# dmar-bonn/ipp-rl

Measured on AMD Instinct MI355X. Metric: env-steps/s (batched) on 50x50 grid, higher is better.
Workload: dtype f32

## Files before the change

ipp-rl_amd/csrc/k_prepare.h:

```cpp
#pragma once
#include "ipp_common.h"

#ifndef IPP_PREP_MINWAVES
#define IPP_PREP_MINWAVES 4
#endif

namespace ipp {

__device__ inline double area_weight(int src, int dst, int d, int s) {
    const double scale = (double)src / (double)dst;
    const double a = d * scale, b = a + scale;
    const double cell = fmin(scale, (double)src - a);
    int s1 = (int)ceil(a);
    const int s2 = min((int)floor(b), src - 1);
    s1 = min(s1, s2);
    double w = 0.0;
    if (s == s1 - 1 && s1 - a > 1e-3) w += (double)(float)((s1 - a) / cell);
    if (s >= s1 && s < s2) w += (double)(float)(1.0 / cell);
    if (s == s2 && b - s2 > 1e-3) w += (double)(float)(fmin(fmin(b - s2, 1.0), cell) / cell);
    return w;
}

template <int MC>
__host__ __device__ constexpr size_t prep_small_bytes() {
// ... 472 lines not shown
    int status = h.status;
    int fallback = 0;

    if (pd) {
        if (tid < m) {
            const int j = tid;
            for (int i = 0; i < m; ++i) Li[i * LD + j] = 0.0;
            Li[j * LD + j] = 1.0 / L[j * LD + j];
            for (int i = j - 1; i >= 0; --i) {
                double s = 0.0;
                for (int k = i + 1; k <= j; ++k) s += L[k * LD + i] * Li[k * LD + j];
                Li[i * LD + j] = -s / L[i * LD + i];
            }
        }
        prep_sync<WAVE>();
        if (tid < m) {
            double s = 0.0;
            for (int i = 0; i <= tid; ++i) s += Li[i * LD + tid] * vv[i];
            yy[tid] = s;
        }
    } else if (MODE == IPP_DENSE) {
        fallback = 1;
        status = IPP_STATUS_CHOL_FALLBACK;
        if (tid == 0) {
            for (int i = 0; i < m; ++i)
                for (int j = 0; j < m; ++j) { L[i * LD + j] = S[i * LD + j]; Li[i * LD + j] = (i == j) ? 1.0 : 0.0; }
            for (int c = 0; c < m; ++c) {
                int piv = c;
                double best = fabs(L[c * LD + c]);
                for (int i = c + 1; i < m; ++i)
                    if (fabs(L[i * LD + c]) > best) { best = fabs(L[i * LD + c]); piv = i; }
                if (piv != c)
                    for (int j = 0; j < m; ++j) {
                        double t = L[c * LD + j]; L[c * LD + j] = L[piv * LD + j]; L[piv * LD + j] = t;
                        t = Li[c * LD + j]; Li[c * LD + j] = Li[piv * LD + j]; Li[piv * LD + j] = t;
                    }
                const double inv = 1.0 / L[c * LD + c];
                for (int j = 0; j < m; ++j) { L[c * LD + j] *= inv; Li[c * LD + j] *= inv; }
                for (int i = 0; i < m; ++i)
                    if (i != c) {
                        const double fct = L[i * LD + c];
                        if (fct != 0.0)
                            for (int j = 0; j < m; ++j) { L[i * LD + j] -= fct * L[c * LD + j]; Li[i * LD + j] -= fct * Li[c * LD + j]; }
                    }
            }
        }
        prep_sync<WAVE>();
        if (tid < m) {
            double s = 0.0;
            for (int i = 0; i < m; ++i) s += Li[tid * LD + i] * vv[i];
            yy[tid] = s;
        }
    } else {
        status = IPP_STATUS_NOT_PD;
    }
    prep_sync<WAVE>();
    IPP_TICK(v, 5, tick);

    if (WAVE && threadIdx.x == 0) IPP_MARK(item, 7);
    const bool dead = (MODE == IPP_FACTOR) && !pd;
    for (int idx = tid; idx < MC * MC; idx += kPrepThreads) {
        const int i = idx / MC, j = idx - i * MC;
        const double val = (!dead && i < m && j < m) ? Li[i * LD + j] : 0.0;
        linv_f[idx] = (float)val;
        if (linv_f2) linv_f2[idx] = (float)val;
        dbg[MC * MC + idx] = val;
        dbg[idx] = (i < m && j < m) ? S[i * LD + j] : 0.0;
    }
    for (int i = tid; i < MC; i += kPrepThreads) {
        const double yval = (!dead && !cov_only && i < m) ? yy[i] : 0.0;
        y_f[i] = (float)yval;
        if (y_f2) y_f2[i] = (float)yval;
        dbg[2 * MC * MC + i] = (i < m) ? zz[i] : 0.0;
        dbg[2 * MC * MC + MC + i] = yval;
    }
    constexpr int QS = (MC + 3) & ~3;
    constexpr int QP = (QS <= 16) ? 16 : 32;
    if (MODE == IPP_FACTOR) {
        const int j = tid & (QP - 1);
        if (j < QS) {
            for (int k = tid / QP; k < r; k += kPrepThreads / QP) {
                double sacc = 0.0;
                const int SI = (si > 0) ? si : ht_ld, SK = (si > 0) ? sk : 1;
                if (!dead && j < m)
                    for (int i = 0; i <= j; ++i) sacc += (double)big[i * SI + k * SK] * Li[i * LD + j];
                q_out[k * QS + j] = (float)(-sacc);
            }
        }
    } else {
        const int j = tid & (QP - 1);
        if (j < QS) {
            for (int fi = tid / QP; fi < f; fi += kPrepThreads / QP) {
                const int ly = fi / h.w, lx = fi - ly * h.w;
                const int bi = (ly / h.rf) * h.nx + lx / h.rf;
                double sacc = 0.0;
                if (j < m) sacc = fallback ? ((bi == j) ? bwt[bi] : 0.0) : bwt[bi] * Li[bi * LD + j];
                q_out[fi * QS + j] = (float)sacc;
            }
        }
    }
    {
        const int qrows = (MODE == IPP_FACTOR) ? r : f;
        for (int idx = tid; idx < 8 * QS; idx += kPrepThreads) q_out[(size_t)qrows * QS + idx] = 0.f;
    }
    if (tid == 0) {
        ItemHdr ho = h;
        ho.status = status;
        ho.fallback = fallback;
        if (dead) { ho.commit = 0; ho.rows = 0; }
        v.hdr[item] = ho;
        *hs = ho;
        if (status_out) status_out[item] = status;
    }
    IPP_TICK(v, 6, tick);
    return hs;
}

template <int MC, int MODE, int NT>
__device__ __forceinline__ ItemHdr* prepare_item(const View& v, const int item, const int* __restrict__ env_ids,
                                                 const int* __restrict__ dst_ids, const double* __restrict__ action,
                                                 const double* __restrict__ prev_action,
                                                 const float* __restrict__ meas_noise, unsigned flags,
                                                 int* __restrict__ status_out, float* __restrict__ obs_out,
                                                 int* __restrict__ obs_m, int* __restrict__ obs_shape,
                                                 unsigned char* small, float* big, int si, int sk, float* q_out,
                                                 float* linv_f, float* linv_f2, float* y_f, float* y_f2, int* span_s) {
    return prepare_item_ex<MC, MODE, NT, false>(v, item, env_ids, dst_ids, action, prev_action, meas_noise, flags, status_out,
                                                obs_out, obs_m, obs_shape, small, big, si, sk, q_out, linv_f, linv_f2, y_f,
                                                y_f2, span_s, NoMidWork());
}

__device__ __forceinline__ void wave_lds_sync() {
    __builtin_amdgcn_fence(__ATOMIC_ACQ_REL, "workgroup");
    __builtin_amdgcn_wave_barrier();
}

template <int MC>
__device__ __forceinline__ int solve_wave(const View& v, const ItemHdr& h, const int item, unsigned flags,
                                          unsigned char* small, const float* ht, float* linv_f, float* y_f,
                                          int* __restrict__ status_out) {
    constexpr int LD = MC + 1;
    constexpr int QS = (MC + 3) & ~3;
    const PrepLds<MC> pl(small);
    double* S = pl.S; double* L = pl.L; double* Li = pl.Li; double* zz = pl.zz; double* vv = pl.vv; double* yy = pl.yy;
    const double* ktab = pl.ktab; const int* bfi = pl.bfi; const int* bcnt = pl.bcnt; const double* bwt = pl.bwt;
    const int lane = threadIdx.x & (kWave - 1);
    const int m = h.m, r = h.rank;
    const double R = (double)(h.rf * h.rf * h.rf) * h.nv_d;
    const bool cov_only = (flags & IPP_COV_ONLY) != 0;
    double* dbg = v.dbg + (size_t)item * (2 * MC * MC + 2 * MC);

    {
        constexpr int GL = 8;
        const int grp = lane / GL, sl = lane & (GL - 1), n_grp = kWave / GL;
        const int npairs = m * (m + 1) / 2;
        for (int p0 = 0; p0 < npairs; p0 += n_grp) {
            const int p = p0 + grp;
            const bool on = p < npairs;
            int i = 0, j = 0;
            if (on) {
                j = (int)((sqrtf(8.0f * p + 1.0f) - 1.0f) * 0.5f);
                while (j * (j + 1) / 2 > p) --j;
                while ((j + 1) * (j + 2) / 2 <= p) ++j;
                i = p - j * (j + 1) / 2;
            }
            double acc = 0.0;
            if (on) {
                const int ci = bcnt[i], cj = bcnt[j];
                const int sh = (cj == 4) ? 2 : (cj == 2 ? 1 : 0);
                const double wij = bwt[i] * bwt[j];
                for (int c = sl; c < ci * cj; c += GL) {
                    const int fa = bfi[4 * i + (c >> sh)], fb = bfi[4 * j + (c & (cj - 1))];
                    acc += wij * ktab[abs(bfi_y(fa) - bfi_y(fb)) * h.w + abs(bfi_x(fa) - bfi_x(fb))];
                }
                for (int k = sl; k < r; k += GL) acc -= (double)ht[k * QS + i] * (double)ht[k * QS + j];
            }
#pragma unroll
            for (int off = GL / 2; off > 0; off >>= 1) acc += __shfl_xor(acc, off, GL);
            if (on && sl == 0) {
                if (i == j) acc += R;
                S[i * LD + j] = acc;
                S[j * LD + i] = acc;
            }
        }
    }
    wave_lds_sync();

    bool pd = true;
    for (int c = 0; c < m; ++c) {
        double d = 0.0;
        if (lane == 0) {
            d = S[c * LD + c];
            for (int k = 0; k < c; ++k) d -= L[c * LD + k] * L[c * LD + k];
            L[c * LD + c] = sqrt(d);
        }
        d = __shfl(d, 0, kWave);
        if (!(d > 0.0)) { pd = false; break; }
        wave_lds_sync();
        if (lane > c && lane < m) {
            double sacc = S[lane * LD + c];
            for (int k = 0; k < c; ++k) sacc -= L[lane * LD + k] * L[c * LD + k];
            L[lane * LD + c] = sacc / L[c * LD + c];
        }
        wave_lds_sync();
    }
    int status = h.status;
    if (pd) {
        if (lane < m) {
            const int j = lane;
            for (int i = 0; i < m; ++i) Li[i * LD + j] = 0.0;
            Li[j * LD + j] = 1.0 / L[j * LD + j];
            for (int i = j - 1; i >= 0; --i) {
                double sacc = 0.0;
                for (int k = i + 1; k <= j; ++k) sacc += L[k * LD + i] * Li[k * LD + j];
                Li[i * LD + j] = -sacc / L[i * LD + i];
            }
        }
        wave_lds_sync();
        if (lane < m) {
            double sacc = 0.0;
            for (int i = 0; i <= lane; ++i) sacc += Li[i * LD + lane] * vv[i];
            yy[lane] = sacc;
        }
        wave_lds_sync();
    } else {
        status = IPP_STATUS_NOT_PD;
    }
    const bool dead = !pd;
    for (int idx = lane; idx < MC * MC; idx += kWave) {
        const int i = idx / MC, j = idx - i * MC;
        const double val = (!dead && i < m && j < m) ? Li[i * LD + j] : 0.0;
        linv_f[idx] = (float)val;
        dbg[MC * MC + idx] = val;
        dbg[idx] = (i < m && j < m) ? S[i * LD + j] : 0.0;
    }
    for (int i = lane; i < MC; i += kWave) {
        const double yval = (!dead && !cov_only && i < m) ? yy[i] : 0.0;
        y_f[i] = (float)yval;
        dbg[2 * MC * MC + i] = (i < m) ? zz[i] : 0.0;
        dbg[2 * MC * MC + MC + i] = yval;
    }
    if (lane == 0) {
        ItemHdr ho = h;
        ho.status = status;
        ho.fallback = 0;
        if (dead) { ho.commit = 0; ho.rows = 0; }
        v.hdr[item] = ho;
        if (status_out) status_out[item] = status;
    }
    return status;
}

template <int MC>
__device__ __forceinline__ void observe_wave(const View& v, const ItemHdr& h, unsigned flags, unsigned char* small, const ObsRegs o) {
    const PrepLds<MC> pl(small);
    double* L = pl.L; double* zz = pl.zz; double* vv = pl.vv; double* sub = pl.sub;
    const int lane = threadIdx.x & (kWave - 1);
    const int m = h.m, f = h.f;
    const bool cov_only = (flags & IPP_COV_ONLY) != 0;
    if (cov_only) {
        if (lane < MC) { zz[lane] = 0.0; vv[lane] = 0.0; }
        wave_lds_sync();
        return;
    }
    float gt_f = o.gt;
    asm volatile("" : "+v"(gt_f));
    if (lane < f) sub[lane] = (double)gt_f;
    double* wyt = L;
    double* wxt = L + 2 * MC;
    if (h.rf > 1) {
        const int ocols = (h.h + h.rf - 1) / h.rf, orows = (h.w + h.rf - 1) / h.rf;
        for (int idx = lane; idx < orows * h.h; idx += kWave) wyt[idx] = area_weight(h.h, orows, idx / h.h, idx % h.h);
        for (int idx = lane; idx < ocols * h.w; idx += kWave) wxt[idx] = area_weight(h.w, ocols, idx / h.w, idx % h.w);
    }
    wave_lds_sync();
    if (lane < m) {
        const Block myb = block_of(lane, h.nx, h.rf, h.w, h.h);
        double val;
        if (h.rf == 1) {
            val = sub[lane];
        } else {
            const int ocols = (h.h + h.rf - 1) / h.rf;
            const int orow = lane / ocols, ocol = lane - orow * ocols;
            val = 0.0;
            for (int sy = 0; sy < h.h; ++sy) {
                const double wy = wyt[orow * h.h + sy];
                if (wy == 0.0) continue;
                for (int sx = 0; sx < h.w; ++sx) {
                    const double wx = wxt[ocol * h.w + sx];
                    if (wx != 0.0) val += sub[sy * h.w + sx] * wx * wy;
                }
            }
        }
        float eps_f = o.eps;
        asm volatile("" : "+v"(eps_f));
        const double eps = (double)eps_f;
        if (flags & IPP_GIVEN_OBSERVATION)
            val = eps;
        else
            val = fmin(fmax(val + h.nv_d * eps, 0.0), 1.0);
        zz[lane] = val;
        double hx = 0.0;
        const int cnt_b = myb.count();
#pragma unroll
        for (int a = 0; a < 4; ++a)
            if (a < cnt_b) hx += myb.weight * (double)o.mean[a];
        vv[lane] = val - hx;
    } else if (lane < MC) {
        zz[lane] = 0.0;
        vv[lane] = 0.0;
    }
    wave_lds_sync();
}


template <int MC>
__device__ __forceinline__ int solve_wave_fast(const View& v, const ItemHdr& h, const int item, unsigned flags,
                                               unsigned char* small, const float* ht, int si, int sk, float* linv_f,
                                               float* y_f, float* __restrict__ q_out, int* __restrict__ status_out,
                                               int* obs_flag = nullptr, int r_ht = -1, const float* ht2 = nullptr, int r_ht2 = 0) {
    static_assert(MC == 9, "register layout written for MC = 9");
    constexpr int LD = MC + 1;
    constexpr int QS = (MC + 3) & ~3;
    const PrepLds<MC> pl(small);
    double* S = pl.S; double* zz = pl.zz; double* vv = pl.vv;
    const double* ktab = pl.ktab; const int* bfi = pl.bfi; const int* bcnt = pl.bcnt; const double* bwt = pl.bwt;
    const int lane = threadIdx.x & (kWave - 1);
    const int m = h.m, r = r_ht >= 0 ? r_ht : h.rank;
    const double R = (double)(h.rf * h.rf * h.rf) * h.nv_d;
    const bool cov_only = (flags & IPP_COV_ONLY) != 0;
    double* dbg = v.dbg + (size_t)item * (2 * MC * MC + 2 * MC);

    int pi = 0, pj = 0;
    {
        int j = (int)((sqrtf(8.0f * lane + 1.0f) - 1.0f) * 0.5f);
        while (j * (j + 1) / 2 > lane) --j;
        while ((j + 1) * (j + 2) / 2 <= lane) ++j;
        pj = j;
        pi = lane - j * (j + 1) / 2;
    }
    const bool pair_on = pj < m;
    double mine = 0.0;
    if (pair_on) {
        const int ci = bcnt[pi], cj = bcnt[pj];
        const int sh = (cj == 4) ? 2 : (cj == 2 ? 1 : 0);
        const double wij = bwt[pi] * bwt[pj];
        for (int c = 0; c < ci * cj; ++c) {
            const int fa = bfi[4 * pi + (c >> sh)], fb = bfi[4 * pj + (c & (cj - 1))];
            mine += wij * ktab[abs(bfi_y(fa) - bfi_y(fb)) * h.w + abs(bfi_x(fa) - bfi_x(fb))];
        }
        if (pi == pj) mine += R;
    }
    if (pair_on) {
        const float* hi = ht + pi * si;
        const float* hj = ht + pj * si;
        double a0 = 0.0, a1 = 0.0, a2 = 0.0, a3 = 0.0;
        auto groups = [&](const float* xi, const float* xj, int n) {
            int k = 0;
            for (; k + 8 <= n; k += 8) {
                float x[8], y[8];
#pragma unroll
                for (int u = 0; u < 8; ++u) { x[u] = xi[(k + u) * sk]; y[u] = xj[(k + u) * sk]; }
                a0 = fma((double)x[0], (double)y[0], a0); a1 = fma((double)x[1], (double)y[1], a1);
                a2 = fma((double)x[2], (double)y[2], a2); a3 = fma((double)x[3], (double)y[3], a3);
                a0 = fma((double)x[4], (double)y[4], a0); a1 = fma((double)x[5], (double)y[5], a1);
                a2 = fma((double)x[6], (double)y[6], a2); a3 = fma((double)x[7], (double)y[7], a3);
            }
            for (; k < n; ++k) a0 = fma((double)xi[k * sk], (double)xj[k * sk], a0);
        };
        groups(hi, hj, r);
        if (ht2) groups(ht2 + pi * si, ht2 + pj * si, r_ht2);
        mine -= (a0 + a1) + (a2 + a3);
    }
    if (pair_on) {
        S[pi * LD + pj] = mine;
        S[pj * LD + pi] = mine;
    }
    wave_lds_sync();

    double c[MC];
#pragma unroll
    for (int k = 0; k < MC; ++k) c[k] = (lane < m && k < m) ? S[min(lane, MC - 1) * LD + k] : ((k == lane) ? 1.0 : 0.0);
    const bool capture = v.dbg_capture == 1;
    if (capture && lane < MC) {
#pragma unroll
        for (int k = 0; k < MC; ++k) dbg[lane * MC + k] = (lane < m && k < m) ? c[k] : 0.0;
    }
    bool pd = true;
    double rd[MC];
#pragma unroll
    for (int j = 0; j < MC; ++j) {
        rd[j] = 1.0;
        if (j < m) {
            double t = c[j];
#pragma unroll
            for (int k = 0; k < j; ++k) t = fma(-c[k], bcast_lane(c[k], j), t);
            const double d = bcast_lane(t, j);
            if (!(d > 0.0)) pd = false;
            double y = __builtin_amdgcn_rsq(d);
#pragma unroll
            for (int it = 0; it < 2; ++it) {
                const double e = fma(-(d * y), y, 1.0);
                y = fma(0.5 * y, e, y);
            }
            rd[j] = y;
            c[j] = (lane == j) ? d * y : t * y;
        }
    }
    int status = h.status;
    double li[MC];
#pragma unroll
    for (int i = 0; i < MC; ++i) li[i] = 0.0;
    if (pd) {
#pragma unroll
        for (int i = MC - 1; i >= 0; --i) {
            if (i < m) {
                double sacc = 0.0;
#pragma unroll
                for (int k = i + 1; k < MC; ++k) {
                    if (k < m) {
                        const double cki = bcast_lane(c[i], k);
                        if (k <= lane) sacc = fma(cki, li[k], sacc);
                    }
                }
                li[i] = (lane == i) ? rd[i] : ((lane > i && lane < m) ? -sacc * rd[i] : 0.0);
            }
        }
    } else {
        status = IPP_STATUS_NOT_PD;
    }
    const bool dead = !pd;
    if (obs_flag) {
        while (__hip_atomic_load(obs_flag, __ATOMIC_ACQUIRE, __HIP_MEMORY_SCOPE_WORKGROUP) == 0) __builtin_amdgcn_s_sleep(2);
    }
    double yv = 0.0;
    if (pd && lane < m) {
#pragma unroll
        for (int i = 0; i < MC; ++i)
            if (i <= lane) yv = fma(li[i], vv[i], yv);
    }
    if (lane < MC) {
#pragma unroll
        for (int i = 0; i < MC; ++i) {
            const double val = (!dead && i < m && lane < m) ? li[i] : 0.0;
            linv_f[i * MC + lane] = (float)val;
            if (capture) dbg[MC * MC + i * MC + lane] = val;
        }
        const double yval = (!dead && !cov_only && lane < m) ? yv : 0.0;
        y_f[lane] = (float)yval;
        if (capture) {
            dbg[2 * MC * MC + lane] = (lane < m) ? zz[lane] : 0.0;
            dbg[2 * MC * MC + MC + lane] = yval;
        }
    }
    if (lane == 0) {
        ItemHdr ho = h;
        ho.status = status;
        ho.fallback = 0;
        if (dead) { ho.commit = 0; ho.rows = 0; }
        v.hdr[item] = ho;
        *pl.hs = ho;
        if (status_out) status_out[item] = status;
    }
    wave_lds_sync();
    if (q_out) {
        for (int k0 = 0; k0 < r; k0 += kWave) {
            const int k = k0 + lane;
            if (k < r) {
                float hv[MC], q[QS];
#pragma unroll
                for (int i = 0; i < MC; ++i) hv[i] = (i < m) ? ht[i * si + k * sk] : 0.f;
#pragma unroll
                for (int j = 0; j < QS; ++j) {
                    float acc = 0.f;
                    if (j < MC) {
#pragma unroll
                        for (int i = 0; i <= j; ++i) acc = fmaf(hv[i], linv_f[i * MC + j], acc);
                    }
                    q[j] = -acc;
                }
                float4* dst = reinterpret_cast<float4*>(q_out + (size_t)k * QS);
#pragma unroll
                for (int j4 = 0; j4 < QS / 4; ++j4) dst[j4] = make_float4(q[4 * j4], q[4 * j4 + 1], q[4 * j4 + 2], q[4 * j4 + 3]);
            }
        }
        for (int idx = lane; idx < 8 * QS; idx += kWave) q_out[(size_t)r * QS + idx] = 0.f;
    }
    return status;
}

template <int MC, int MODE>
__global__ __launch_bounds__(kPrepThreads, IPP_PREP_MINWAVES) void k_prepare(View v, const int* __restrict__ env_ids,
                                                          const int* __restrict__ dst_ids, int n_items,
                                                          const double* __restrict__ action,
                                                          const double* __restrict__ prev_action,
                                                          const float* __restrict__ meas_noise, unsigned flags,
                                                          int* __restrict__ status_out, float* __restrict__ obs_out,
                                                          int* __restrict__ obs_m, int* __restrict__ obs_shape) {
    extern __shared__ __attribute__((aligned(16))) unsigned char smem[];
    if ((int)blockIdx.x >= n_items) return;
    const int item = launch_item(v, blockIdx.x, n_items);
    constexpr int LQ = (MC * MC + MC + 3) & ~3;
    float* blk_out = v.q + (size_t)item * v.q_item;
    float* big = reinterpret_cast<float*>(smem + ((prep_small_bytes<MC>() + 15) & ~(size_t)15));
    if constexpr (MC == 9 && MODE == IPP_FACTOR) {
        if (!obs_out) {
            ItemHdr* hs = prepare_item_ex<MC, MODE, kPrepThreads, true>(v, item, env_ids, dst_ids, action, prev_action, meas_noise, flags,
                                                                        status_out, nullptr, nullptr, nullptr, smem, big, 0, 1, nullptr,
                                                                        v.linv + (size_t)item * MC * MC, blk_out, v.yv + (size_t)item * MC,
                                                                        blk_out + MC * MC, nullptr, NoMidWork());
            if (threadIdx.x >= kWave) return;
            const ItemHdr h = uniform_hdr(*hs);
            if (h.m == 0) return;
            const PrepLds<MC> pl(smem);
            float* Ls = reinterpret_cast<float*>(pl.L);
            float* ys = Ls + MC * MC;
            solve_wave_fast<MC>(v, h, item, flags, smem, big, (h.rank + 3) & ~3, 1, Ls, ys, blk_out + LQ, status_out);
            wave_lds_sync();
            const int lane = threadIdx.x;
            for (int i = lane; i < MC * MC; i += kWave) { const float x = Ls[i]; v.linv[(size_t)item * MC * MC + i] = x; blk_out[i] = x; }
            if (lane < MC) { const float x = ys[lane]; v.yv[(size_t)item * MC + lane] = x; blk_out[MC * MC + lane] = x; }
            return;
        }
    }
    prepare_item<MC, MODE, kPrepThreads>(v, item, env_ids, dst_ids, action, prev_action, meas_noise, flags, status_out,
                                         obs_out, obs_m, obs_shape, smem, big, 0, 1, blk_out + LQ,
                                         v.linv + (size_t)item * MC * MC, blk_out, v.yv + (size_t)item * MC,
                                         blk_out + MC * MC, nullptr);
}

}
```

ipp-rl_amd/csrc/k_step_patch.h:

```cpp
#pragma once
#include <algorithm>
#include <cstdlib>
#include <type_traits>
#include "ipp_common.h"
#include "k_gain.h"
#include "k_gain_factor.h"
#include "k_prepare.h"

namespace ipp {

constexpr int kPatchRec = 16;
constexpr int kPatchKP = 8;
constexpr int kPatchRowAux = 2;
constexpr int kPatchStoreAux = IPP_NT_STORES ? 2 : 0;
constexpr int kPatchMinW = 6;
constexpr int kPatchWavesDefault = 3;
constexpr int kPatchWavesPerCu = 4 * kPatchMinW;
constexpr int kPatchCtl = 32;
constexpr int kPatchMaxRank = 512;

struct PatchGeo {
    int pw, ph, pstride, plw, punits;
};
inline PatchGeo patch_geometry(int W, int H, int R) {
    PatchGeo g;
    g.pw = std::min((W + 1) & ~1, ((2 * R + 5 + 2) / 2) * 2);
    g.ph = std::min(H, 2 * R + 6);
    g.pstride = (g.pw * g.ph + 15) & ~15;
    g.plw = std::min(std::max(W, H), R + 7);
    g.punits = (g.ph * g.pw + 2 * kWave - 1) / (2 * kWave);
    return g;
}

struct PatchLds {
    float* rec; float* Ls; float* ys; float* lut; unsigned char* small; double* red; int* ctl; int* fb_yx; float* fb_w;
    unsigned short* ridx; double* unit_red;
    static constexpr int LQ = 96;
    __host__ __device__ static size_t small_bytes() { return (prep_small_bytes<9>() + 15) & ~(size_t)15; }
    __host__ __device__ static size_t bytes(int cap, int lut_floats, int waves, int units, int rank_cap) {
        size_t b = (size_t)cap * kPatchRec * 4 + LQ * 4 + (size_t)((lut_floats + 3) & ~3) * 4 + small_bytes();
        b += 4 * 8 + kPatchCtl * 4 + 2 * 4 * 9 * 4;
        b += (((size_t)waves * (rank_cap + kPatchKP) * 2) + 15) & ~(size_t)15;
        b += (size_t)units * 8;
        return (b + 15) & ~(size_t)15;
    }
    __device__ __forceinline__ PatchLds(unsigned char* base, int cap, int lut_floats, int waves, int units, int rank_cap) {
        rec = reinterpret_cast<float*>(base);
        Ls = rec + (size_t)cap * kPatchRec;
        ys = Ls + 81;
        lut = Ls + LQ;
        small = reinterpret_cast<unsigned char*>(lut + ((lut_floats + 3) & ~3));
        red = reinterpret_cast<double*>(small + small_bytes());
        ctl = reinterpret_cast<int*>(red + 4);
        fb_yx = ctl + kPatchCtl;
        fb_w = reinterpret_cast<float*>(fb_yx + 4 * 9);
        ridx = reinterpret_cast<unsigned short*>(fb_w + 4 * 9);
        unit_red = reinterpret_cast<double*>(ridx + ((((size_t)waves * (rank_cap + kPatchKP)) + 7) & ~(size_t)7));
    }
};

}
#include "k_patch_units.h"
namespace ipp {

struct StepIo {
    static constexpr bool kMean = true;
    typedef float rowv __attribute__((ext_vector_type(2)));
    __amdgpu_buffer_rsrc_t row_rs;
    float* mean_rw;
    float* diag_rw;
    bool cov_only;
    int m, row0_bytes, pstride_bytes;
    __device__ __forceinline__ rowv row_load(unsigned cofs, unsigned voff) const {
        return __builtin_bit_cast(rowv, __builtin_amdgcn_raw_buffer_load_b64(row_rs, voff, (int)cofs, kPatchRowAux));
    }
    __device__ __forceinline__ float coef(const UnitLds& ul, int a, int l15) const { return ul.rec[(size_t)a * kPatchRec + l15]; }
    __device__ __forceinline__ void load_pre(int cell0, int flat, int rrow, int rcol, float (&md)[2][2]) const {
        load_vec<2>(mean_rw + cell0, md[0]);
        load_vec<2>(diag_rw + cell0, md[1]);
    }
    __device__ __forceinline__ void store(bool commit, bool lane_valid, int cell0, int flat, unsigned flat4, const float (&acc)[2][9],
                                          const float (&md)[2][2], const float (&dred)[2], const float (&dmean)[2]) const {
        if (!commit) return;
        if (lane_valid) {
            float od[2], om[2];
#pragma unroll
            for (int c = 0; c < 2; ++c) { od[c] = md[1][c] - dred[c]; om[c] = md[0][c] + dmean[c]; }
            store_vec<2>(diag_rw + cell0, od);
            if (!cov_only) store_vec<2>(mean_rw + cell0, om);
        }
        typedef decltype(__builtin_amdgcn_raw_buffer_load_b64(row_rs, 0, 0, 0)) raw2;
#pragma unroll
        for (int j = 0; j < 9; ++j)
            if (j < m) {
                rowv t;
#pragma unroll
                for (int c = 0; c < 2; ++c) t[c] = acc[c][j];
                __builtin_amdgcn_raw_buffer_store_b64(__builtin_bit_cast(raw2, t), row_rs, lane_valid ? flat4 : 0xffffffffu, row0_bytes + j * pstride_bytes, kPatchStoreAux);
            }
    }
};

__device__ __forceinline__ bool ledger_done(const Ledger& L, double bud, int dep, double cost) {
    return !(dep + 1 < L.max_steps && bud - cost >= L.res);
}

__device__ __forceinline__ void ledger_close(const View& v, const AutoReset& ar, unsigned flags, int env, int item, int pos, double bud,
                                             int dep, double cost, int lane) {
    const Ledger& L = ar.led;
    const bool done = ledger_done(L, bud, dep, cost);
    const bool rs = done && (flags & IPP_RESET_ON_DONE);
    if (rs) wave_reset_env(v, ar, env, 0, lane);
    if (lane == 0) {
        L.done[item] = done ? 1 : 0;
        if (rs) {
            const long long ep = L.episode[env] + 1;
            L.episode[env] = ep;
            L.budget[env] = budget_start(L, env, ep);
            L.depth[env] = 0;
        } else {
            L.budget[env] = bud - cost;
            L.depth[env] = dep + 1;
        }
        if (flags & IPP_RESET_ON_DONE) L.refill[pos] = rs ? env : -1;
    }
}

template <int NW, int KPN = kPatchKP, int MINW = kPatchMinW, int RJN = 0, bool BUD = false>
__global__ __launch_bounds__(64 * NW, MINW) void k_step_patch(
    View v, const int* __restrict__ env_ids, int n_items, const double* __restrict__ action,
    const double* __restrict__ prev_action, const float* __restrict__ meas_noise, unsigned flags,
    int* __restrict__ status_out, float* __restrict__ reward_out, AutoReset ar) {
    constexpr int MC = 9, VEC = 2, NT = kWave * NW, KP = KPN;
    static_assert(KPN <= kPatchKP, "the row lists are padded for kPatchKP entries");
    static_assert(NW >= 2, "wave 0 runs the m x m algebra, wave 1 the observation");
    constexpr int RJ = RJN > 0 ? RJN : (kPatchMaxRank + NT - 1) / NT;
    constexpr int OW = 1;
    constexpr int TW = (NW > 2) ? 2 : OW;
    extern __shared__ __attribute__((aligned(16))) unsigned char smem_sp[];
    const PatchLds lds(smem_sp, v.pcap, v.plw * v.plw, NW, v.punits, v.rank_cap);
    if ((int)blockIdx.x >= n_items) return;
    const int item = launch_item(v, blockIdx.x, n_items);
    const int tid = threadIdx.x, lane = tid & (kWave - 1), wave = tid / kWave;
    if (tid == 0) IPP_MARK(item, 0);
    IPP_WT_DECL;
    int* next_unit = lds.ctl; int* done_waves = lds.ctl + 1; int* solve_flag = lds.ctl + 2; int* obs_flag = lds.ctl + 3;
    int* wcnt = lds.ctl + 8;

    const int env0 = env_ids ? env_ids[item] : item + v.env_base;
    const bool slots_ok = env0 >= 0 && env0 < v.cap;
    const int envc = slots_ok ? env0 : 0;
    const double ax = action[3 * item + 0], ay = action[3 * item + 1], az = action[3 * item + 2];
    const double px = prev_action[3 * item + 0], py = prev_action[3 * item + 1], pz = prev_action[3 * item + 2];
    const int rank_ld = v.rank[envc];
    const double sv_d = v.prior[2 * envc + 0], ls_d = v.prior[2 * envc + 1];
    const int otid = tid - kWave * OW;
    const float eps_ld = (meas_noise && otid >= 0 && otid < MC) ? meas_noise[(size_t)item * MC + otid] : 0.f;
    double bud_ld = 0.0;
    int dep_ld = 0;
    if constexpr (BUD) { bud_ld = ar.led.budget[envc]; dep_ld = ar.led.depth[envc]; }
    const int* __restrict__ rects = v.colrect + (size_t)envc * v.rank_cap;
    unsigned rc_pre[RJ];
#pragma unroll
    for (int j = 0; j < RJ; ++j) {
        const int k = tid + j * NT;
        rc_pre[j] = (k < v.rank_cap) ? (unsigned)rects[k] : 0u;
    }

    const int R = v.window_rows;
    const PrepLds<MC> pl(lds.small);
    ItemHdr h;
    if (__builtin_amdgcn_readfirstlane(wave) == 0) {
        h = make_item_header<MC, IPP_FACTOR>(v, env0, env0, slots_ok, ax, ay, az, px, py, pz, rank_ld, sv_d, ls_d, flags);
        const int r0 = max(0, h.yu - R), r1 = min(v.H - 1, h.yd + R);
        const int c0 = max(0, h.xl - R) & ~(VEC - 1), c1 = min(v.W - 1, min(v.W - 1, h.xr + R) | (VEC - 1));
        if (h.m > 0 && (r1 - r0 + 1 > v.ph || c1 - c0 + 1 > v.pw)) {
            h.status = IPP_STATUS_BAD_FOOTPRINT; h.m = 0; h.f = 0; h.rows = 0; h.commit = 0;
        }
        if (tid == 0) {
            *pl.hs = h;
            *next_unit = 0; *done_waves = 0; *solve_flag = 0; *obs_flag = 0;
            lds.red[0] = 0.0; lds.red[1] = 0.0;
        }
    }
    __syncthreads();
    if (__builtin_amdgcn_readfirstlane(wave) != 0) h = *pl.hs;
    h = uniform_hdr(h);
    IPP_EXIT_POINT(1);
    const int r0n = max(0, h.yu - R), r1n = min(v.H - 1, h.yd + R);
    const int c0n = max(0, h.xl - R) & ~(VEC - 1), c1n = min(v.W - 1, min(v.W - 1, h.xr + R) | (VEC - 1));
    const int hn = r1n - r0n + 1, wn = c1n - c0n + 1;
    const int m = h.m, f = h.f, r = h.rank;
    if (m == 0) {
        if (tid == 0) {
            v.hdr[item] = h;
            if (status_out) status_out[item] = h.status;
            reward_out[item] = 0.f;
        }
        __syncthreads();
        if ((flags & IPP_UPDATE_PREV) && tid == 0) {
            double* pw = const_cast<double*>(prev_action);
            pw[3 * item + 0] = ax; pw[3 * item + 1] = ay; pw[3 * item + 2] = az;
        }
        if (ar.src && tid < kWave) {
            const int k = __builtin_amdgcn_readfirstlane(ar.src[item]);
            if (k >= 0 && h.env >= 0 && h.env < v.cap) wave_reset_env(v, ar, h.env, k, tid);
        }
        if constexpr (BUD) {
            if (tid < kWave) ledger_close(v, ar, flags, h.env, item, v.pos0 + (int)blockIdx.x, bud_ld, dep_ld, h.cost_d, tid);
        }
        return;
    }
    if (tid == 0) IPP_MARK(item, 3);
    const bool cov_only = (flags & IPP_COV_ONLY) != 0;
    const float* mean_env = v.mean + (size_t)h.env * v.Npad;
    const float* gt_env = gt_plane(v, h.env);
    float* slot = v.cov + (size_t)h.env * v.cov_slot;
    const int cap = v.pcap, pw = v.pw;
    float* ovf = v.q + (size_t)item * v.q_item;

    ObsRegs oregs;
    {
        const int ly = div_small(max(otid, 0), h.w), lx = max(otid, 0) - ly * h.w;
        oregs.gt = (!cov_only && otid >= 0 && otid < f) ? gt_env[(h.yu + ly) * v.W + h.xl + lx] : 0.f;
        const Block mob = block_of(min(max(otid, 0), m - 1), h.nx, h.rf, h.w, h.h);
#pragma unroll
        for (int a = 0; a < 4; ++a) {
            const int aa = min(a, mob.count() - 1);
            const int cell = (h.yu + mob.y0 + blk_dy(aa, mob.bw)) * v.W + h.xl + mob.x0 + blk_dx(aa, mob.bw);
            oregs.mean[a] = (!cov_only && otid >= 0 && otid < m && a < mob.count()) ? mean_env[cell] : 0.f;
        }
        oregs.eps = eps_ld;
    }

    bool con[RJ];
    unsigned long long bal[RJ];
#pragma unroll
    for (int j = 0; j < RJ; ++j) {
        const int k = tid + j * NT;
        const unsigned rc = rc_pre[j];
        const int r0k = rc & 0xff, r1k = (rc >> 8) & 0xff, c0k = (rc >> 16) & 0xff, c1k = rc >> 24;
        con[j] = k < r && r0k <= h.yd && r1k >= h.yu && c0k <= h.xr && c1k >= h.xl;
        bal[j] = __ballot(con[j]);
        if (lane == 0) wcnt[j * NW + wave] = __popcll(bal[j]);
    }
    const int ttid = tid - kWave * TW;
    if (ttid >= 0 && ttid < MC) {
        const Block bb = block_of(min(ttid, m - 1), h.nx, h.rf, h.w, h.h);
        for (int a = 0; a < 4; ++a) {
            const int aa = min(a, bb.count() - 1);
            const int ly = bb.y0 + blk_dy(aa, bb.bw), lx = bb.x0 + blk_dx(aa, bb.bw);
            lds.fb_yx[4 * ttid + a] = (h.yu + ly) | ((h.xl + lx) << 16);
            lds.fb_w[4 * ttid + a] = (ttid < m && a < bb.count()) ? (float)bb.weight : 0.f;
            if (ttid < m) pl.bfi[4 * ttid + a] = bfi_pack(ly, lx, h.w);
        }
        if (ttid < m) { pl.bcnt[ttid] = bb.count(); pl.bwt[ttid] = bb.weight; }
    }
    __syncthreads();
    if (tid == 0) IPP_MARK(item, 4);
    IPP_EXIT_POINT(2);
    int pos[RJ];
    int n_c = 0;
#pragma unroll
    for (int j = 0; j < RJ; ++j) {
        int before = 0, all = 0;
#pragma unroll
        for (int w = 0; w < NW; ++w) {
            const int c = wcnt[j * NW + w];
            before += (w < wave) ? c : 0;
            all += c;
        }
        pos[j] = n_c + before + __popcll(bal[j] & ((1ull << lane) - 1ull));
        n_c += all;
    }
    unsigned short* klist = lds.ridx;
    unsigned* rclist = reinterpret_cast<unsigned*>(pl.S);
    static_assert(4 * kPatchMaxRank <= (3 * MC * (MC + 1) + 3 * MC + 2 * 4 * MC) * 8, "rectangle list does not fit the fp64 scratch");
#pragma unroll
    for (int j = 0; j < RJ; ++j)
        if (con[j]) { klist[pos[j]] = (unsigned short)(tid + j * NT); rclist[pos[j]] = rc_pre[j]; }
    __syncthreads();
    static_assert(4 * kPatchMaxRank <= (3 * MC * (MC + 1) + 3 * MC + 4 * MC) * 8, "rectangle list reaches pl.ktab");

    const int wave_u = __builtin_amdgcn_readfirstlane(wave);
    auto mine = [&](int i) { return (i % NW) == wave_u; };
    const auto slot_rs = __builtin_amdgcn_make_buffer_rsrc(slot, 0, 0x7ffffff0, 0x00020000);
    const auto row_rs = __builtin_amdgcn_make_buffer_rsrc(slot - v.pstride, 0, 0x7ffffff0, 0x00020000);
    auto gather_issue = [&](unsigned rc, int k, bool on, float (&l)[MC][4]) {
        const unsigned first = on ? (rc & 0x00ff00ffu) : 0xffffffffu;
        const unsigned extent = on ? (((rc >> 8) & 0x00ff00ffu) - (rc & 0x00ff00ffu)) : 0u;
        const int base4 = (k * v.pstride - (int)(rc & 0xff) * pw - (int)((rc >> 16) & 0xff)) * 4;
        typedef unsigned short us2g __attribute__((ext_vector_type(2)));
#pragma unroll
        for (int i = 0; i < MC; ++i) {
#pragma unroll
            for (int a = 0; a < 4; ++a) l[i][a] = 0.f;
            if (i < m && mine(i)) {
                const int cnt = uni(pl.bcnt[i]);
#pragma unroll
                for (int a = 0; a < 4; ++a) {
                    if (a < cnt) {
                        const unsigned yx = (unsigned)uni(lds.fb_yx[4 * i + a]);
                        const int cell4 = (int)((yx & 0xffffu) * (unsigned)pw + (yx >> 16)) * 4;
                        const us2g d = __builtin_bit_cast(us2g, yx) - __builtin_bit_cast(us2g, first);
                        const bool in = __builtin_bit_cast(unsigned, __builtin_elementwise_min(d, __builtin_bit_cast(us2g, extent))) == __builtin_bit_cast(unsigned, d);
                        const unsigned voff = in ? (unsigned)(base4 + cell4) : 0xffffffffu;
                        l[i][a] = __builtin_bit_cast(float, __builtin_amdgcn_raw_buffer_load_b32(slot_rs, voff, 0, 0));
                    }
                }
            }
        }
        __builtin_amdgcn_sched_barrier(0);
    };
    auto gather_store = [&](unsigned rc, int k, bool on, int a_pos, const float (&l)[MC][4]) {
        if (!on) return;
        float* dst = (a_pos < cap) ? lds.rec + (size_t)a_pos * kPatchRec : nullptr;
        float* gdst = (a_pos >= cap) ? ovf + (size_t)(a_pos - cap) * kPatchRec : nullptr;
#pragma unroll
        for (int i = 0; i < MC; ++i) {
            if (i < m && mine(i)) {
                const int cnt = uni(pl.bcnt[i]);
                float t = l[i][0];
                if (cnt > 1) t += l[i][1];
                if (cnt > 2) t += l[i][2] + l[i][3];
                const float val = -(t * lds.fb_w[4 * i]);
                if (dst) dst[i] = val;
                if (gdst) gdst[i] = val;
            }
        }
        if (wave_u != 0) return;
#pragma unroll
        for (int i = 0; i < 12; ++i)
            if (i >= m) {
                if (dst) dst[i] = 0.f;
                if (gdst) gdst[i] = 0.f;
            }
        const int r0k = rc & 0xff, r1k = (rc >> 8) & 0xff, c0k = (rc >> 16) & 0xff, c1k = rc >> 24;
        const int shift = (r0n - r0k) * pw + (c0n - c0k);
        const float4 meta = make_float4(__int_as_float((k * v.pstride + shift + v.pstride) * 4),
                                        __int_as_float(r0k | (c0k << 16)),
                                        __int_as_float((r1k - r0k) | ((c1k - c0k) << 16)),
                                        __int_as_float(k));
        if (dst) reinterpret_cast<float4*>(dst)[3] = meta;
        if (gdst) reinterpret_cast<float4*>(gdst)[3] = meta;
    };
    {
        float l0[MC][4];
        const bool any0 = n_c > 0;
        const bool on0 = lane < n_c;
        const int k0 = on0 ? (int)klist[lane] : 0;
        const unsigned rc0 = on0 ? rclist[lane] : 0u;
        if (any0) gather_issue(rc0, k0, on0, l0);
        {
            const float s3 = prior_scale_f(v.prior_kind, v.res, h.ls);
            const int lw = v.plw;
            with_prior_kind(v.prior_kind, [&](auto kind) {
                for (int i = tid; i < lw * lw; i += NT) {
                    const int dr = div_small(i, lw), dc = i - dr * lw;
                    lds.lut[i] = prior_f<decltype(kind)::value>(dr, dc, s3, h.sv);
                }
            });
            if (ttid >= 0 && ttid < f) { const int ky = div_small(ttid, h.w); pl.ktab[ttid] = prior_d(v.prior_kind, ky, ttid - ky * h.w, v.res, sv_d, ls_d); }
        }
        if (tid == 0) IPP_MARK(item, 5);
        if (any0) gather_store(rc0, k0, on0, lane, l0);
    }
#pragma unroll 1
    for (int t0 = kWave; t0 < n_c; t0 += kWave) {
        const int t = t0 + lane;
        const bool on = t < n_c;
        const int kk = on ? (int)klist[t] : 0;
        const unsigned rc = on ? rclist[t] : 0u;
        float l[MC][4];
        gather_issue(rc, kk, on, l);
        gather_store(rc, kk, on, t, l);
    }
    if ((flags & IPP_UPDATE_PREV) && tid == 0) {
        double* pwr = const_cast<double*>(prev_action);
        pwr[3 * item + 0] = ax; pwr[3 * item + 1] = ay; pwr[3 * item + 2] = az;
    }
    const int n_lds = min(n_c, cap), n_ovf = n_c - n_lds;
    if (n_ovf > 0) asm volatile("s_waitcnt vmcnt(0)" ::: "memory");
    __syncthreads();
    if (tid == 0) IPP_MARK(item, 1);
    IPP_WT(6);
    IPP_EXIT_POINT(3);

    int status_w0 = 0;
    if (wave == 0) {
        status_w0 = solve_wave_fast<MC>(v, h, item, flags, lds.small, lds.rec, 1, kPatchRec, lds.Ls, lds.ys, nullptr, status_out,
                                        obs_flag, n_lds, n_ovf > 0 ? ovf : nullptr, n_ovf);
        __builtin_amdgcn_fence(__ATOMIC_RELEASE, "workgroup");
        if (lane == 0) __hip_atomic_store(solve_flag, status_w0 == IPP_STATUS_NOT_PD ? 2 : 1, __ATOMIC_RELEASE, __HIP_MEMORY_SCOPE_WORKGROUP);
        if (lane == 0) IPP_MARK(item, 7);
    } else if (wave == OW) {
        observe_wave<MC>(v, h, flags, lds.small, oregs);
        __builtin_amdgcn_fence(__ATOMIC_RELEASE, "workgroup");
        if (lane == 0) __hip_atomic_store(obs_flag, 1, __ATOMIC_RELEASE, __HIP_MEMORY_SCOPE_WORKGROUP);
    }
    IPP_WT(7);
    IPP_EXIT_POINT(4);
    const UnitGeo ug = unit_geometry(r0n, c0n, hn, wn);
    const int n_units = ug.n_units;

    const int n_fast = min(n_lds, 2 * kWave);
    unsigned mcofs[2], mlo[2], mex[2];
#pragma unroll
    for (int p2 = 0; p2 < 2; ++p2) {
        const int a = p2 * kWave + lane;
        mcofs[p2] = 0u; mlo[p2] = 0x0000ffffu; mex[p2] = 0u;
        if (a < n_fast) {
            const float4 mt = *reinterpret_cast<const float4*>(lds.rec + (size_t)a * kPatchRec + 12);
            mcofs[p2] = __float_as_uint(mt.x); mlo[p2] = __float_as_uint(mt.y); mex[p2] = __float_as_uint(mt.z);
        }
    }

    const bool commit_u = h.commit != 0;
    const int env_u = h.env;
    StepIo io;
    io.row_rs = row_rs;
    io.mean_rw = v.mean + (size_t)env_u * v.Npad;
    io.diag_rw = v.diag + (size_t)env_u * v.Npad;
    io.cov_only = cov_only;
    io.m = m;
    io.row0_bytes = (r + 1) * v.pstride * 4;
    io.pstride_bytes = v.pstride * 4;
    UnitArgs ua;
    ua.m = m; ua.rf1 = (h.rf == 1); ua.adaptive = (flags & IPP_ADAPTIVE) != 0; ua.commit_u = commit_u;
    ua.n_c = n_c; ua.n_fast = n_fast; ua.cap = cap; ua.ovf = ovf;
    ua.next_unit = next_unit; ua.solve_flag = solve_flag; ua.item = item;
    ua.ridx = lds.ridx + (size_t)wave * (v.rank_cap + KP);
    const UnitLds ul = {lds.rec, lds.Ls, lds.ys, lds.lut, lds.fb_yx, lds.fb_w};
    unsigned long long units = 0, needed = 0;
    bool dead = false;
    patch_units<KP>(v, ul, lds.unit_red, io, ua, ug, mcofs, mlo, mex, units, needed, dead);
    IPP_EXIT_POINT(5);
    IPP_WT_RESET;
    IPP_WT_COUNT(11, 1);

    unsigned long long* cnt = reinterpret_cast<unsigned long long*>(lds.red);
    if (lane == 0 && units) { atomicAdd(cnt, units); atomicAdd(cnt + 1, needed); }
    int reset_k = -1;
    if (ar.src) reset_k = __builtin_amdgcn_readfirstlane(ar.src[item]);
    if constexpr (BUD) {
        if ((flags & IPP_RESET_ON_DONE) && ledger_done(ar.led, bud_ld, dep_ld, pl.hs->cost_d)) reset_k = 0;
    }
    if (reset_k >= 0) asm volatile("s_waitcnt vmcnt(0)" ::: "memory");
    __builtin_amdgcn_fence(__ATOMIC_RELEASE, "workgroup");
    int arrived = 0;
    if (lane == 0) arrived = atomicAdd(done_waves, 1);
    arrived = __builtin_amdgcn_readfirstlane(arrived);
    if (arrived == 0 && lane == 0) IPP_MARK(item, 6);
    if (arrived != NW - 1) { IPP_WT_FLUSH(lane); return; }
    __builtin_amdgcn_fence(__ATOMIC_ACQUIRE, "workgroup");
    dead = __hip_atomic_load(solve_flag, __ATOMIC_ACQUIRE, __HIP_MEMORY_SCOPE_WORKGROUP) == 2;
    const bool commit_item = commit_u && !dead;
    const double cost_d = pl.hs->cost_d;
    const int t_span = pl.hs->t_lo | (pl.hs->t_hi << 16);
    if (lane == 0) {
        IPP_MARK(item, 2);
        double tot = 0.0;
        for (int t = 0; t < n_units; ++t) tot += lds.unit_red[t];
        reward_out[item] = dead ? NAN : (float)(tot / (cost_d + 1.0));
        if (commit_item) v.rank[env_u] = r + m;
        if (cnt[0]) {
            unsigned long long* ic = v.item_counts + 2 * (size_t)item;
            atomicAdd(ic, cnt[0]);
            atomicAdd(ic + 1, cnt[1]);
        }
    }
    if (commit_item && lane < m) {
        v.colspan[(size_t)env_u * v.rank_cap + r + lane] = t_span;
        v.colrect[(size_t)env_u * v.rank_cap + r + lane] = (int)rect_pack(r0n, r1n, c0n, c1n);
    }
    if constexpr (BUD) ledger_close(v, ar, flags, env_u, item, v.pos0 + (int)blockIdx.x, bud_ld, dep_ld, cost_d, lane);
    else if (reset_k >= 0) wave_reset_env(v, ar, env_u, reset_k, lane);
    IPP_WT(8);
    IPP_WT_FLUSH(lane);
}

__global__ __launch_bounds__(256) void k_read_cov_patch(View v, int env, float* __restrict__ out) {
    const int i = blockIdx.y;
    const int j = blockIdx.x * blockDim.x + threadIdx.x;
    if (i >= v.N || j >= v.N) return;
    const double sv = v.prior[2 * env + 0], ls = v.prior[2 * env + 1];
    const int ri = i / v.W, ci = i - ri * v.W, rj = j / v.W, cj = j - rj * v.W;
    double acc = prior_d(v.prior_kind, ri - rj, ci - cj, v.res, sv, ls);
    const float* U = v.cov + (size_t)env * v.cov_slot;
    const int r = v.rank[env];
    for (int k = 0; k < r; ++k) {
        const unsigned rc = (unsigned)v.colrect[(size_t)env * v.rank_cap + k];
        if (!rect_has(rc, ri, ci) || !rect_has(rc, rj, cj)) continue;
        const int r0 = rc & 0xff, c0 = (rc >> 16) & 0xff;
        const float* p = U + (size_t)k * v.pstride;
        acc -= (double)p[(ri - r0) * v.pw + (ci - c0)] * (double)p[(rj - r0) * v.pw + (cj - c0)];
    }
    out[(size_t)i * v.N + j] = (float)acc;
}

}
```

Measured before the change: 56.75 million.

## Precompute gather sites per lane and use buffer loads for observation reads

Each lane now precomputes one block-site offset for the patch gather, and the gather loops read these offsets with readlane. This replaces per-iteration LDS reads and modulo ownership checks. A fast path for rf==1 issues only the first of each block's four loads. Observation gt and mean loads now run only on the observing wave, through raw buffer loads with out-of-range offsets so masked lanes need no branches. The gt slot load is hoisted ahead of the barrier, and an explicit waitcnt plus an asm barrier on the mean values control instruction scheduling.

```diff
diff --git a/ipp-rl_amd/csrc/k_prepare.h b/ipp-rl_amd/csrc/k_prepare.h
--- a/ipp-rl_amd/csrc/k_prepare.h
+++ b/ipp-rl_amd/csrc/k_prepare.h
@@ -798,9 +798,12 @@
         zz[lane] = val;
         double hx = 0.0;
         const int cnt_b = myb.count();
+        float mean_f[4];
+#pragma unroll
+        for (int a = 0; a < 4; ++a) { mean_f[a] = o.mean[a]; asm volatile("" : "+v"(mean_f[a])); }
 #pragma unroll
         for (int a = 0; a < 4; ++a)
-            if (a < cnt_b) hx += myb.weight * (double)o.mean[a];
+            if (a < cnt_b) hx += myb.weight * (double)mean_f[a];
         vv[lane] = val - hx;
     } else if (lane < MC) {
         zz[lane] = 0.0;
diff --git a/ipp-rl_amd/csrc/k_step_patch.h b/ipp-rl_amd/csrc/k_step_patch.h
--- a/ipp-rl_amd/csrc/k_step_patch.h
+++ b/ipp-rl_amd/csrc/k_step_patch.h
@@ -153,6 +153,7 @@
     const double ax = action[3 * item + 0], ay = action[3 * item + 1], az = action[3 * item + 2];
     const double px = prev_action[3 * item + 0], py = prev_action[3 * item + 1], pz = prev_action[3 * item + 2];
     const int rank_ld = v.rank[envc];
+    const int gt_slot_ld = v.gt_slot[envc];
     const double sv_d = v.prior[2 * envc + 0], ls_d = v.prior[2 * envc + 1];
     const int otid = tid - kWave * OW;
     const float eps_ld = (meas_noise && otid >= 0 && otid < MC) ? meas_noise[(size_t)item * MC + otid] : 0.f;
@@ -184,6 +185,7 @@
         }
     }
     __syncthreads();
+    __builtin_amdgcn_s_waitcnt(0x0f70);
     if (__builtin_amdgcn_readfirstlane(wave) != 0) h = *pl.hs;
     h = uniform_hdr(h);
     IPP_EXIT_POINT(1);
@@ -214,23 +216,30 @@
     if (tid == 0) IPP_MARK(item, 3);
     const bool cov_only = (flags & IPP_COV_ONLY) != 0;
     const float* mean_env = v.mean + (size_t)h.env * v.Npad;
-    const float* gt_env = gt_plane(v, h.env);
+    const float* gt_env = v.gt + (size_t)gt_slot_ld * v.Npad;
     float* slot = v.cov + (size_t)h.env * v.cov_slot;
     const int cap = v.pcap, pw = v.pw;
     float* ovf = v.q + (size_t)item * v.q_item;
 
     ObsRegs oregs;
-    {
-        const int ly = div_small(max(otid, 0), h.w), lx = max(otid, 0) - ly * h.w;
-        oregs.gt = (!cov_only && otid >= 0 && otid < f) ? gt_env[(h.yu + ly) * v.W + h.xl + lx] : 0.f;
-        const Block mob = block_of(min(max(otid, 0), m - 1), h.nx, h.rf, h.w, h.h);
+    oregs.gt = 0.f;
+    oregs.eps = eps_ld;
+#pragma unroll
+    for (int a = 0; a < 4; ++a) oregs.mean[a] = 0.f;
+    if (__builtin_amdgcn_readfirstlane(wave) == OW && !cov_only) {
+        const auto gt_rs = __builtin_amdgcn_make_buffer_rsrc(const_cast<float*>(gt_env), 0, v.N * 4, 0x00020000);
+        const auto mean_rs = __builtin_amdgcn_make_buffer_rsrc(const_cast<float*>(mean_env), 0, v.N * 4, 0x00020000);
+        const int ly = div_small(otid, h.w), lx = otid - ly * h.w;
+        const unsigned gofs = otid < f ? (unsigned)((h.yu + ly) * v.W + h.xl + lx) * 4u : 0xffffffffu;
+        oregs.gt = __builtin_bit_cast(float, __builtin_amdgcn_raw_buffer_load_b32(gt_rs, gofs, 0, 0));
+        const Block mob = block_of(min(otid, m - 1), h.nx, h.rf, h.w, h.h);
 #pragma unroll
         for (int a = 0; a < 4; ++a) {
             const int aa = min(a, mob.count() - 1);
             const int cell = (h.yu + mob.y0 + blk_dy(aa, mob.bw)) * v.W + h.xl + mob.x0 + blk_dx(aa, mob.bw);
-            oregs.mean[a] = (!cov_only && otid >= 0 && otid < m && a < mob.count()) ? mean_env[cell] : 0.f;
-        }
-        oregs.eps = eps_ld;
+            const unsigned mofs = (otid < m && a < mob.count()) ? (unsigned)cell * 4u : 0xffffffffu;
+            oregs.mean[a] = __builtin_bit_cast(float, __builtin_amdgcn_raw_buffer_load_b32(mean_rs, mofs, 0, 0));
+        }
     }
 
     bool con[RJ];
@@ -283,46 +292,63 @@
     static_assert(4 * kPatchMaxRank <= (3 * MC * (MC + 1) + 3 * MC + 4 * MC) * 8, "rectangle list reaches pl.ktab");
 
     const int wave_u = __builtin_amdgcn_readfirstlane(wave);
-    auto mine = [&](int i) { return (i % NW) == wave_u; };
+    constexpr int NB = (MC + NW - 1) / NW;
+    static_assert(4 * NB <= kWave, "one request site per lane");
+    const bool rf1 = h.rf == 1;
+    unsigned site_yx, site_c4;
+    {
+        const int sj = lane >> 2, sa = lane & 3, si = wave_u + NW * sj;
+        const bool s_on = si < m && sa < pl.bcnt[min(si, MC - 1)];
+        site_yx = s_on ? (unsigned)lds.fb_yx[4 * min(si, MC - 1) + sa] : 0x80008000u;
+        site_c4 = ((site_yx & 0xffffu) * (unsigned)pw + (site_yx >> 16)) * 4u;
+    }
     const auto slot_rs = __builtin_amdgcn_make_buffer_rsrc(slot, 0, 0x7ffffff0, 0x00020000);
     const auto row_rs = __builtin_amdgcn_make_buffer_rsrc(slot - v.pstride, 0, 0x7ffffff0, 0x00020000);
-    auto gather_issue = [&](unsigned rc, int k, bool on, float (&l)[MC][4]) {
+    auto gather_issue = [&](unsigned rc, int k, bool on, float (&l)[NB][4]) {
         const unsigned first = on ? (rc & 0x00ff00ffu) : 0xffffffffu;
         const unsigned extent = on ? (((rc >> 8) & 0x00ff00ffu) - (rc & 0x00ff00ffu)) : 0u;
         const int base4 = (k * v.pstride - (int)(rc & 0xff) * pw - (int)((rc >> 16) & 0xff)) * 4;
         typedef unsigned short us2g __attribute__((ext_vector_type(2)));
-#pragma unroll
-        for (int i = 0; i < MC; ++i) {
-#pragma unroll
-            for (int a = 0; a < 4; ++a) l[i][a] = 0.f;
-            if (i < m && mine(i)) {
-                const int cnt = uni(pl.bcnt[i]);
-#pragma unroll
-                for (int a = 0; a < 4; ++a) {
-                    if (a < cnt) {
-                        const unsigned yx = (unsigned)uni(lds.fb_yx[4 * i + a]);
-                        const int cell4 = (int)((yx & 0xffffu) * (unsigned)pw + (yx >> 16)) * 4;
-                        const us2g d = __builtin_bit_cast(us2g, yx) - __builtin_bit_cast(us2g, first);
-                        const bool in = __builtin_bit_cast(unsigned, __builtin_elementwise_min(d, __builtin_bit_cast(us2g, extent))) == __builtin_bit_cast(unsigned, d);
-                        const unsigned voff = in ? (unsigned)(base4 + cell4) : 0xffffffffu;
-                        l[i][a] = __builtin_bit_cast(float, __builtin_amdgcn_raw_buffer_load_b32(slot_rs, voff, 0, 0));
-                    }
-                }
-            }
+        auto site_off = [&](int s) {
+            const unsigned yx = (unsigned)__builtin_amdgcn_readlane((int)site_yx, s);
+            const int cell4 = __builtin_amdgcn_readlane((int)site_c4, s);
+            const us2g d = __builtin_bit_cast(us2g, yx) - __builtin_bit_cast(us2g, first);
+            const bool in = __builtin_bit_cast(unsigned, __builtin_elementwise_min(d, __builtin_bit_cast(us2g, extent))) == __builtin_bit_cast(unsigned, d);
+            return in ? (unsigned)(base4 + cell4) : 0xffffffffu;
+        };
+        auto request = [&](unsigned voff) { return __builtin_bit_cast(float, __builtin_amdgcn_raw_buffer_load_b32(slot_rs, voff, 0, 0)); };
+        unsigned v0[NB];
+#pragma unroll
+        for (int j = 0; j < NB; ++j) v0[j] = site_off(4 * j);
+#pragma unroll
+        for (int j = 0; j < NB; ++j) l[j][0] = request(v0[j]);
+        if (!rf1) {
+            unsigned v1[NB][3];
+#pragma unroll
+            for (int j = 0; j < NB; ++j)
+#pragma unroll
+                for (int a = 1; a < 4; ++a) v1[j][a - 1] = site_off(4 * j + a);
+#pragma unroll
+            for (int j = 0; j < NB; ++j)
+#pragma unroll
+                for (int a = 1; a < 4; ++a) l[j][a] = request(v1[j][a - 1]);
         }
         __builtin_amdgcn_sched_barrier(0);
     };
-    auto gather_store = [&](unsigned rc, int k, bool on, int a_pos, const float (&l)[MC][4]) {
+    auto gather_store = [&](unsigned rc, int k, bool on, int a_pos, const float (&l)[NB][4]) {
         if (!on) return;
         float* dst = (a_pos < cap) ? lds.rec + (size_t)a_pos * kPatchRec : nullptr;
         float* gdst = (a_pos >= cap) ? ovf + (size_t)(a_pos - cap) * kPatchRec : nullptr;
 #pragma unroll
-        for (int i = 0; i < MC; ++i) {
-            if (i < m && mine(i)) {
-                const int cnt = uni(pl.bcnt[i]);
-                float t = l[i][0];
-                if (cnt > 1) t += l[i][1];
-                if (cnt > 2) t += l[i][2] + l[i][3];
+        for (int j = 0; j < NB; ++j) {
+            const int i = wave_u + NW * j;
+            if (i < m) {
+                float t = l[j][0];
+                if (!rf1) {
+                    const int cnt = uni(pl.bcnt[i]);
+                    if (cnt > 1) t += l[j][1];
+                    if (cnt > 2) t += l[j][2] + l[j][3];
+                }
                 const float val = -(t * lds.fb_w[4 * i]);
                 if (dst) dst[i] = val;
                 if (gdst) gdst[i] = val;
@@ -345,7 +371,7 @@
         if (gdst) reinterpret_cast<float4*>(gdst)[3] = meta;
     };
     {
-        float l0[MC][4];
+        float l0[NB][4];
         const bool any0 = n_c > 0;
         const bool on0 = lane < n_c;
         const int k0 = on0 ? (int)klist[lane] : 0;
@@ -371,7 +397,7 @@
         const bool on = t < n_c;
         const int kk = on ? (int)klist[t] : 0;
         const unsigned rc = on ? rclist[t] : 0u;
-        float l[MC][4];
+        float l[NB][4];
         gather_issue(rc, kk, on, l);
         gather_store(rc, kk, on, t, l);
     }
```

After: 57.90 million (median of 5 runs). 1.02x the previous value.
